# ASSERT-KTH/QuantizedSAE

Measured on AMD Instinct MI355X. Metric: activations/sec, BinarySAE 512->32768 n_bits=4 forward (dense latent + reconstruction + MSE), higher is better.
Workload: dtype f32; 1 GPU; BinarySAE(512, 32768, gamma=4.0, n_bits=4) k=65, 65536 rows per GPU per step, reference forward() signature (dense [B,32768] latent, [B,512] reconstruction, polarize loss) + recon-MSE accumulation; rows_per_gpu=65536, input_dim=512, hidden_dim=32768, n_bits=4, top_k=65, parallelism=row-sharded x1, no data-path collective, batches_in_flight=2

## Files before the change

### quantizedsae_amd/csrc/encode_topk_internal.h

```cpp
#pragma once

#include "gemm_mfma_f32_dma.h"
#include "decode_row.h"

namespace qsae {

int topk_rows_dispatch(float* latent, int64_t ld, int B, int H, int k, int32_t* idx, float* val, int zero_rest,
                       float* tau, uint2* cand, int* cnt, int cap, float* dense, int64_t dense_ld, hipStream_t s,
                       const float* margin = nullptr, int stride = 0);
int scatter_rows(const int32_t* idx, const float* val, int B, int k, int H, float* dense, int64_t ld, hipStream_t s);
int decode_binary_sparse_rows(const int* rows, int nrows, const int32_t* idx, const float* val, int k, int H,
                              const RowDecode& d, hipStream_t s);
int densify_rows(const int32_t* idx, const float* val, int B, int k, int H, float* dense, int64_t ld, hipStream_t s);
int gather_rows(const float* src, const int* rows, int n, int D, float* dst, hipStream_t s);
void launch_x_prep(const float* x, int B, int D, const float* meta, _Float16* xq, float* inv, float* margin, hipStream_t s,
                   int* zero_word = nullptr);

constexpr int kChunkRows = 1024;
constexpr int kTopkMaxH = 32768;
constexpr int kCandCap = 1024;
constexpr int kMaxSpecRows = kChunkRows;
constexpr int kRefMaxD = 2048;
constexpr int kRefTileStride = 36;

#ifdef QSAE_DEBUG_BUILD
#define QSAE_TUNABLE int
#define QSAE_TUNABLE_PTR unsigned long long*
extern int kPilotRank, g_xstat_rot, g_ref_ablate, g_ref_sliced, g_x_phase;
extern unsigned long long* g_ref_stamps;
#else
#define QSAE_TUNABLE static constexpr int
#define QSAE_TUNABLE_PTR static constexpr unsigned long long*
#endif
#if !defined(QSAE_DEBUG_BUILD) || defined(QSAE_DEFINE_SHARED_TUNABLES)
QSAE_TUNABLE kPilotRank = 20;
QSAE_TUNABLE g_xstat_rot = 2;
QSAE_TUNABLE_PTR g_ref_stamps = nullptr;
QSAE_TUNABLE g_ref_ablate = 0;
#ifdef QSAE_AB_NO_SLICED
QSAE_TUNABLE g_ref_sliced = 0;
#else
QSAE_TUNABLE g_ref_sliced = 1;
#endif
QSAE_TUNABLE g_x_phase = 3;
#endif

static inline size_t align_up(size_t v, size_t a) { return (v + a - 1) / a * a; }
bool use_fused(int B, int D, int H, int k);
int pilot_width(int H);

struct FusedLayout {
    size_t pilot, tau, cnt, cnt_split, cand, flags, fx, flat, fidx, fval, fpart, total;
};
FusedLayout fused_layout(int B, int D, int H, int k);

template <int BM, int BN, int WMW = 2, int WNW = 2, bool APPROX = false>
struct EpiFilter : EpiTile<BM, BN, WMW, WNW> {
    using T = EpiTile<BM, BN, WMW, WNW>;
    static constexpr int MT = T::MT, NT = T::NT;
    static constexpr int kThreads = 64 * WMW * WNW;
    static constexpr int kLdsFloats = BN;
    static constexpr int kStoresPerFinish = (BM * BN * 4) / (kThreads * 16);
    struct Args {
        const float* bias;
        const float* tau;
        uint2* cand;
        int* cnt;
        int cap;
        int hidden_offset;
        float* dense;
        int64_t dense_ld;
        const float* inv;
        const float* margin;
        int parts = 1;
        int* cnt_parts = nullptr;
    };
    float tau[NT];
    float inv[NT];
    bool col_ok[NT];

    __device__ __forceinline__ void begin(const Args& a, const TileCtx& c) {
        int* counters = reinterpret_cast<int*>(c.lds_epi);
        if (c.tid < BN) {
            const int row = c.n0 + c.tid;
            counters[c.tid] = (row < c.N && c.part == 0) ? a.cnt[row] : 0;
        }
#pragma unroll
        for (int nt = 0; nt < NT; ++nt) {
            const int col = T::col(c, nt);
            col_ok[nt] = col < c.N;
            tau[nt] = col_ok[nt] ? a.tau[col] : __builtin_huge_valf();
            inv[nt] = 1.0f;
            if (APPROX && col_ok[nt]) {
                tau[nt] = tau[nt] - a.margin[col];
                inv[nt] = a.inv[col];
            }
        }
    }
    __device__ __forceinline__ void init(const Args& a, f32x16 (&acc)[MT][NT], const TileCtx& c) {
#pragma unroll
        for (int mt = 0; mt < MT; ++mt)
#pragma unroll
            for (int r = 0; r < 16; ++r) {
                int h = T::row(c, mt, r);
                h = h < c.M ? h : c.M - 1;
                const float b = (!APPROX && a.bias) ? a.bias[h] : 0.0f;
#pragma unroll
                for (int nt = 0; nt < NT; ++nt) acc[mt][nt][r] = b;
            }
    }
    __device__ __forceinline__ void finish(const Args& a, f32x16 (&acc)[MT][NT], const TileCtx& c) {
        int* counters = reinterpret_cast<int*>(c.lds_epi);
        if (a.dense != nullptr) {
            constexpr int CPR = BM / 4;
            const int h0 = c.m0 + a.hidden_offset;
            const f32x4 z = {0.f, 0.f, 0.f, 0.f};
#pragma unroll
            for (int i = 0; i < (BN * CPR) / kThreads; ++i) {
                const int chunk = i * kThreads + c.tid;
                const int row = c.n0 + chunk / CPR, cc = 4 * (chunk % CPR);
                if (row < c.N && (c.m0 + cc) < c.M)
                    *reinterpret_cast<f32x4*>(a.dense + static_cast<int64_t>(row) * a.dense_ld + h0 + cc) = z;
            }
        }
        float hb[MT][16];
        if (APPROX) {
// ... 56 lines not shown
```

### quantizedsae_amd/csrc/prefilter_topk.hip

```cpp
#ifdef QSAE_DEBUG_BUILD
#define QSAE_DEFINE_SHARED_TUNABLES 1
#endif
#include "encode_topk_internal.h"
#include "sweep_xstat_f16.h"
#include "refine_row.h"
#include "refine_sliced.h"

namespace qsae {

constexpr int kFillCoWaves = 1024;
constexpr int kFillCoPace = 3;

QSAE_TUNABLE_PTR g_xstat_stamps = nullptr;
QSAE_TUNABLE g_fuse_xprep = 0;
QSAE_TUNABLE g_inkernel_pilot = 1;
QSAE_TUNABLE g_inkernel_rank = 0;
QSAE_TUNABLE g_pilot_tile = 0;
QSAE_TUNABLE g_fill_in_sweep = 1;
QSAE_TUNABLE g_fill_co = 1;
QSAE_TUNABLE g_xstat_ablate = 0;
QSAE_TUNABLE g_x_parts = 0;
QSAE_TUNABLE g_pref_tile = 2;

struct PrefLayout {
    size_t xq, inv, margin, cnt_parts, sl_offs, total_extra;
};
static PrefLayout pref_layout(int B, int D, size_t base) {
    PrefLayout P;
    size_t off = base;
    P.xq = off;     off = align_up(off + static_cast<size_t>(B) * D * 2, 256);
    P.inv = off;    off = align_up(off + static_cast<size_t>(B) * 4, 256);
    P.margin = off; off = align_up(off + static_cast<size_t>(B) * 4, 256);
    P.cnt_parts = off; off = align_up(off + static_cast<size_t>(B) * 4 * 7, 256);
    P.sl_offs = off; off = align_up(off + static_cast<size_t>(B) * 65, 256);
    P.total_extra = off;
    return P;
}

__global__ void __launch_bounds__(256)
pref_w_stats_kernel(const float* __restrict__ W, const float* __restrict__ bias, int H, int D, unsigned* __restrict__ meta) {
    const int row = blockIdx.x * 4 + (threadIdx.x >> 6), lane = threadIdx.x & 63;
    if (row >= H) return;
    float mx = 0.f, ss = 0.f;
    for (int d = lane; d < D; d += 64) pref_w_stat_step(W[static_cast<int64_t>(row) * D + d], mx, ss);
    pref_w_stat_join(mx, ss);
    if (lane == 0) {
        const float nrm = pref_w_row_norm(ss);
        atomicMax(&meta[1], __float_as_uint(nrm));
        atomicMax(&meta[3], __float_as_uint(mx));
        if (bias) atomicMax(&meta[2], __float_as_uint(fabsf(bias[row])));
    }
}

__global__ void __launch_bounds__(256)
pref_w_cast_kernel(const float* __restrict__ W, long long n, float* __restrict__ meta, _Float16* __restrict__ Wq) {
    const float sw = pow2_scale_for(meta[3]);
    const long long gid = static_cast<long long>(blockIdx.x) * blockDim.x + threadIdx.x;
    if (gid == 0) meta[0] = sw;
    if (gid < n) Wq[gid] = pref_w_cast(W[gid], sw);
}

__global__ void __launch_bounds__(256)
pref_w_err_kernel(const float* __restrict__ W, int H, int D, const float* __restrict__ sw_ptr, unsigned* __restrict__ out) {
    const int row = blockIdx.x * 4 + (threadIdx.x >> 6), lane = threadIdx.x & 63;
    if (row >= H) return;
    const float sw = *sw_ptr;
    if (!(sw > 0.f)) return;
    const float back = 1.0f / sw;
    float ff = 0.f;
    for (int d = lane; d < D; d += 64) pref_w_err_step(W[static_cast<int64_t>(row) * D + d], sw, back, ff);
    ff = pref_w_err_join(ff);
    if (lane == 0) atomicMax(out, __float_as_uint(pref_w_row_err(ff)));
}

template <int NV>
__global__ void __launch_bounds__(256)
pref_x_prep_kernel(const float* __restrict__ x, int B, int D, const float* __restrict__ meta,
                   _Float16* __restrict__ xq, float* __restrict__ inv, float* __restrict__ margin, int* __restrict__ zero_word) {
    const int row = blockIdx.x * 4 + (threadIdx.x >> 6), lane = threadIdx.x & 63;
    if (zero_word && blockIdx.x == 0 && threadIdx.x == 0) *zero_word = 0;
    if (row >= B) return;
    const float* xr = x + static_cast<int64_t>(row) * D;
    _Float16* qr = xq + static_cast<int64_t>(row) * D;
    float mx = 0.f, ss = 0.f;
    f32x4 keep[NV > 0 ? NV : 1];
    if (NV > 0) {
#pragma unroll
        for (int j = 0; j < NV; ++j) keep[j] = *reinterpret_cast<const f32x4*>(xr + 256 * j + 4 * lane);
#pragma unroll
        for (int j = 0; j < NV; ++j)
#pragma unroll
            for (int e = 0; e < 4; ++e) {
                const float v = keep[j][e], a = fabsf(v);
                mx = (a > mx || a != a) ? a : mx;
                ss = fmaf(v, v, ss);
            }
    } else {
        for (int d = lane; d < D; d += 64) {
            const float v = xr[d];
            const float a = fabsf(v);
            mx = (a > mx || a != a) ? a : mx;
            ss = fmaf(v, v, ss);
        }
    }
    for (int off = 32; off > 0; off >>= 1) {
        const float o = __shfl_xor(mx, off, 64);
        mx = (o > mx || o != o) ? o : mx;
        ss += __shfl_xor(ss, off, 64);
    }
    const float sx0 = pow2_scale_for(mx), back = sx0 > 0.f ? 1.0f / sx0 : 0.f;
    float ee = 0.f;
    if (NV > 0) {
#pragma unroll
        for (int j = 0; j < NV; ++j) {
            typedef _Float16 f16x4 __attribute__((ext_vector_type(4)));
            f16x4 q;
#pragma unroll
// ... 195 lines not shown
    const SweepProfile prof = take_sweep_profile();
    const PrefPlan pl = pref_plan(c);
    const FusedLayout& L = pl.L;
    const PrefLayout& PL = pl.PL;
    const int B = c.B, D = c.D, H = c.H, k = c.k, P = pl.P;
    char* ws = c.ws;
    float* pilot = reinterpret_cast<float*>(ws + L.pilot);
    float* tau = reinterpret_cast<float*>(ws + L.tau);
    int* cnt = reinterpret_cast<int*>(ws + L.cnt);
    uint2* cand = reinterpret_cast<uint2*>(ws + L.cand);
    int* flags = reinterpret_cast<int*>(ws + L.flags);
    _Float16* xq = reinterpret_cast<_Float16*>(ws + PL.xq);
    float* inv = reinterpret_cast<float*>(ws + PL.inv);
    float* margin = reinterpret_cast<float*>(ws + PL.margin);
    int* cnt_parts = reinterpret_cast<int*>(ws + PL.cnt_parts);
    const bool xstat = pl.xstat, inkernel = pl.inkernel, fill_co = pl.fill_co, fill_in_sweep = pl.fill_in_sweep;
    float* fused_fill = xstat ? nullptr : c.dense;
    const int Hs = pl.Hs, hoff = pl.hoff, parts = pl.parts, cap_part = pl.cap_part;
    const int xs_iters = xstat ? (Hs / kXsHT) / parts + (inkernel ? P / kXsHT : 0) : 0;
    const int fill_cw = xs_iters > 0 ? (32 * (H / 256) / parts + xs_iters - 1) / xs_iters : 0;
    ThreadDeviceCtx* ctx = nullptr;
    if (fill_co) {
        const int rc0 = thread_device_ctx(&ctx);
        if (rc0 != QSAE_OK) return rc0;
    }
    const bool fuse_prep = inkernel && g_fuse_xprep;
    if (!fuse_prep && (g_x_phase & 1)) {
        launch_x_prep(c.x, B, D, c.meta, xq, inv, margin, s, flags);
        QSAE_LAUNCH_CHECK();
    } else {
        QSAE_HIP(hipMemsetAsync(flags, 0, sizeof(int), s));
    }
    const int Kw = D / 2;
    const float* xq_w = reinterpret_cast<const float*>(xq);
    const float* wq_w = reinterpret_cast<const float*>(c.Wq);
    int rc = QSAE_OK;
    if (!inkernel) {
        if (g_pilot_tile == 0 && P % 256 == 0) {
            using EpiP = EpiApproxDense<256, 256, 4, 2>;
            typename EpiP::Args ep{inv, c.bias, pilot, P};
            rc = launch_gemm_dma<EpiP, 256, 256, true, 2>(xq_w, B, wq_w, P, Kw, ep, s, 8);
        } else {
            using EpiP = EpiApproxDense<256, 128, 4, 2>;
            typename EpiP::Args ep{inv, c.bias, pilot, P};
            rc = launch_gemm_dma<EpiP, 256, 128, true>(xq_w, B, wq_w, P, Kw, ep, s, 8);
        }
        if (rc != QSAE_OK) return rc;
    }
    const int j = kPilotRank < P ? kPilotRank : P;
    if (!inkernel) rc = topk_rows_dispatch(pilot, P, B, P, j, nullptr, nullptr, 0, tau, cand, cnt, cap_part, fused_fill, c.dense_ld, s,
                                margin, kCandCap);
    if (rc != QSAE_OK) return rc;
    if (g_x_phase & 1) {
        using EpiS = EpiFilter<256, 128, 4, 2, true>;
        typename EpiS::Args es{c.bias ? c.bias + P : nullptr, tau, cand, cnt, kCandCap, P, fused_fill, c.dense_ld, inv, margin};
        if (prof.begin) QSAE_HIP(hipEventRecord(prof.begin, s));
        if (xstat) {
            XsArgs xa{};
            xa.xq = xq;  xa.wq = c.Wq + static_cast<size_t>(hoff) * D;  xa.bias = c.bias ? c.bias + hoff : nullptr;  xa.tau = tau;
            xa.margin = margin;  xa.inv = inv;  xa.cand = cand;  xa.cnt = cnt;  xa.B = B;  xa.Hs = Hs;  xa.cap = kCandCap;
            xa.hidden_offset = hoff;  xa.rot_mul = g_xstat_rot;  xa.stamps = g_xstat_stamps;  xa.H = H;  xa.fill_cw = fill_cw;
            xa.dense = fill_in_sweep ? c.dense : nullptr;  xa.dense_ld = c.dense_ld;  xa.pilot_stages = inkernel ? P / kXsHT : 0;
            xa.pilot_rank = g_inkernel_rank > 0 ? g_inkernel_rank : inkernel_rank(k);  xa.tau_out = tau;  xa.meta = c.meta;
            xa.x32 = fuse_prep ? c.x : nullptr;  xa.inv_out = inv;  xa.margin_out = margin;  xa.parts = parts;  xa.cnt_parts = cnt_parts;
            if (fill_co) QSAE_HIP(hipEventRecord(ctx->ev_fork, s));
            rc = launch_xstat(D, xa, s, (g_xstat_ablate == 0 && D == 512 && !fill_in_sweep) ? 9 : g_xstat_ablate);
            if (fill_co && rc == QSAE_OK) rc = launch_fill_co(ctx, c.dense, c.dense_ld, B, H, s);
        } else if (g_pref_tile != 1) {
            using EpiW = EpiFilter<256, 256, 4, 2, true>;
            typename EpiW::Args ew{es.bias, es.tau, es.cand, es.cnt, es.cap, es.hidden_offset, es.dense, es.dense_ld, es.inv,
                                   es.margin};
            rc = launch_gemm_dma<EpiW, 256, 256, true, 2>(wq_w + static_cast<size_t>(P) * Kw, H - P, xq_w, B, Kw, ew, s);
        } else {
            rc = launch_gemm_dma<EpiS, 256, 128, true>(wq_w + static_cast<size_t>(P) * Kw, H - P, xq_w, B, Kw, es, s);
        }
        if (prof.end) QSAE_HIP(hipEventRecord(prof.end, s));
        if (rc != QSAE_OK) return rc;
        if (xstat && g_xstat_ablate != 0) return QSAE_OK;
    }
    if (g_x_phase & 2) {
        const RowDecode rd = c.dec ? *c.dec : RowDecode{nullptr, 0, 0, 0, 0, 0.f, nullptr, nullptr, nullptr};
        if (refine_sliced_wanted(B, D, H, k))
            return launch_refine_sliced(cand, cnt, tau, margin, c.x, c.W, c.bias, B, D, H, k, c.idx, c.val, flags, pl.filled, c.dense_ld,
                                        parts, cnt_parts, reinterpret_cast<uint8_t*>(ws + PL.sl_offs), rd, s);
        return launch_refine_row(cand, cnt, tau, margin, c.x, c.W, c.bias, B, D, H, k, c.idx, c.val, flags, pl.filled, c.dense_ld, parts,
                                 cnt_parts, rd, s);
    }
    QSAE_LAUNCH_CHECK();
    return QSAE_OK;
}

static FlaggedArgs pref_flagged_args(const PrefCall& c, const PrefPlan& pl) {
    return FlaggedArgs{c.x, c.W, c.bias, c.B, c.D, c.H, c.k, c.idx, c.val, c.ws, pl.L, c.stream, false,
                       pl.filled, c.dense_ld};
}

static int prefilter_finish(const PrefCall& c, int first, int nflag) {
    hipStream_t s = as_stream(c.stream);
    const PrefPlan pl = pref_plan(c);
    if (pl.xstat && g_xstat_ablate != 0) return QSAE_OK;
    if (nflag < 0 || nflag > c.B) return fail(QSAE_ERR_INVALID_ARG, "%s: flagged-row count out of range", __func__);
    int rc = flagged_range(pref_flagged_args(c, pl), first, nflag);
    if (rc != QSAE_OK) return rc;
    if (c.dec && nflag > 0) {
        const int* flags = reinterpret_cast<const int*>(c.ws + pl.L.flags);
        rc = decode_binary_sparse_rows(flags + 1, nflag, c.idx, c.val, c.k, c.H, *c.dec, s);
        if (rc != QSAE_OK) return rc;
    }
    if (c.dense && !pl.filled)
        return pl.xstat ? densify_rows(c.idx, c.val, c.B, c.k, c.H, c.dense, c.dense_ld, s)
                        : scatter_rows(c.idx, c.val, c.B, c.k, c.H, c.dense, c.dense_ld, s);
    return QSAE_OK;
}

static int run_prefilter(const PrefCall& c, int spec, int* flagged_rows) {
    int rc = prefilter_submit(c);
    if (rc != QSAE_OK) return rc;
    const PrefPlan pl = pref_plan(c);
    if (pl.xstat && g_xstat_ablate != 0) return QSAE_OK;
    const FlaggedArgs fa = pref_flagged_args(c, pl);
    int nflag = 0;
    hipStream_t s = as_stream(c.stream);
    {
        const int* flags = reinterpret_cast<const int*>(c.ws + pl.L.flags);
        ThreadDeviceCtx* ctx = nullptr;
        rc = thread_device_ctx(&ctx);
        if (rc != QSAE_OK) return rc;
        *ctx->pinned = 0;
        QSAE_HIP(hipMemcpyAsync(ctx->pinned, flags, sizeof(int), hipMemcpyDeviceToHost, s));
        QSAE_HIP(hipEventRecord(ctx->ev_copied, s));
        spec = spec < 0 ? 0 : (spec > kMaxSpecRows ? kMaxSpecRows : spec);
        spec = spec < c.B ? spec : c.B;
        rc = flagged_spec(fa, spec);
        if (rc != QSAE_OK) return rc;
        QSAE_HIP(hipEventSynchronize(ctx->ev_copied));
        nflag = *ctx->pinned;
    }
    if (flagged_rows) *flagged_rows = nflag;
    return prefilter_finish(c, spec, nflag);
}

}

using namespace qsae;

#ifdef QSAE_DEBUG_BUILD
namespace qsae { extern int g_pilot_div, g_force_path, g_sweep_kernel; }
extern "C" int qsae_debug_set_xstat_stamps(void* buf) {
    g_xstat_stamps = static_cast<unsigned long long*>(buf);
    return QSAE_OK;
}

extern "C" int qsae_debug_set_refine_stamps(void* buf) {
    g_ref_stamps = static_cast<unsigned long long*>(buf);
    return QSAE_OK;
}

extern "C" int qsae_debug_set_refine_sliced(int v) {
    g_ref_sliced = v;
    return QSAE_OK;
}

extern "C" int qsae_debug_set_refine_ablate(int v) {
    g_ref_ablate = v;
    return QSAE_OK;
}

extern "C" int qsae_debug_set_pilot(int div, int rank) {
    g_pilot_div = div;
    kPilotRank = rank;
    return QSAE_OK;
}

extern "C" int qsae_debug_set_inkernel_pilot(int enable, int rank) {
    g_fuse_xprep = enable >= 2 ? 1 : 0;
    enable = enable ? 1 : 0;
    g_inkernel_pilot = enable;
    g_inkernel_rank = rank;
    return QSAE_OK;
}

extern "C" int qsae_debug_set_fill_co(int v) {
    g_fill_co = v;
    return QSAE_OK;
}

extern "C" int qsae_debug_set_xstat_rot(int rot) {
    g_pilot_tile = rot >= 1000 ? 1 : 0;
    rot %= 1000;
    g_fill_in_sweep = rot >= 100 ? 0 : 1;
    rot %= 100;
    g_xstat_rot = rot;
    return QSAE_OK;
}

extern "C" int qsae_debug_set_prefilter_tile(int which) {
    g_xstat_ablate = which >= 10 ? which - 10 : 0;
    g_pref_tile = which >= 10 ? 2 : which;
    return QSAE_OK;
}

extern "C" int qsae_debug_set_phases(int phase_mask, int parts) {
    g_x_phase = phase_mask;
    g_x_parts = parts;
    return QSAE_OK;
}

extern "C" int qsae_debug_set_sweep_kernel(int which) {
    g_sweep_kernel = which;
    return QSAE_OK;
}

extern "C" int qsae_debug_set_topk_path(int path) {
    g_force_path = path;
    return QSAE_OK;
}

extern "C" int qsae_debug_prefilter_offsets(int B, int D, int H, int k, size_t* pilot_off, size_t* margin_off,
                                            int* pilot_cols) {
    const FusedLayout L = fused_layout(B, D, H, k);
    const PrefLayout PL = pref_layout(B, D, L.total);
    if (pilot_off) *pilot_off = L.pilot;
    if (margin_off) *margin_off = PL.margin;
    if (pilot_cols) *pilot_cols = pilot_width(H);
    return QSAE_OK;
}

extern "C" int qsae_debug_prefilter_list_offsets(int B, int D, int H, int k, size_t* cand_off, size_t* cnt_off,
                                                 size_t* cnt_parts_off, size_t* tau_off, size_t* margin_off, int* cap,
                                                 int* parts) {
    const FusedLayout L = fused_layout(B, D, H, k);
    const PrefLayout PL = pref_layout(B, D, L.total);
    if (cand_off) *cand_off = L.cand;
    if (cnt_off) *cnt_off = L.cnt;
    if (cnt_parts_off) *cnt_parts_off = PL.cnt_parts;
    if (tau_off) *tau_off = L.tau;
    if (margin_off) *margin_off = PL.margin;
    if (cap) *cap = kCandCap;
    if (parts) *parts = xstat_parts(B, H, kCandCap);
    return QSAE_OK;
}
#endif

extern "C" double qsae_profile_sweep_flop_fraction(int H) {
    if (H <= 0) return 0.0;
    if (g_inkernel_pilot && g_pref_tile == 2 && H % kXsHT == 0 && pilot_width(H) % kXsHT == 0) return 1.0;
    return static_cast<double>(H - pilot_width(H)) / static_cast<double>(H);
}

extern "C" size_t qsae_prefilter_w_bytes(int H, int D) {
    return (H > 0 && D > 0) ? static_cast<size_t>(H) * D * 2 : 0;
}

extern "C" int qsae_prefilter_pack_w(const float* W, const float* bias, int H, int D, void* Wq, float* meta,
                                     qsae_stream_t stream) {
    QSAE_CHECK_ARG(H > 0 && D > 0 && W && Wq && meta, "H > 0, D > 0, non-null pointers");
    hipStream_t s = as_stream(stream);
    QSAE_HIP(hipMemsetAsync(meta, 0, 4 * sizeof(float), s));
    hipLaunchKernelGGL(pref_w_stats_kernel, dim3((H + 3) / 4), dim3(256), 0, s, W, bias, H, D,
                       reinterpret_cast<unsigned*>(meta));
    QSAE_LAUNCH_CHECK();
    const long long n = static_cast<long long>(H) * D;
    hipLaunchKernelGGL(pref_w_cast_kernel, dim3(static_cast<unsigned>((n + 255) / 256)), dim3(256), 0, s, W, n, meta,
                       static_cast<_Float16*>(Wq));
    QSAE_LAUNCH_CHECK();
    QSAE_HIP(hipMemsetAsync(meta + 3, 0, sizeof(float), s));
    hipLaunchKernelGGL(pref_w_err_kernel, dim3((H + 3) / 4), dim3(256), 0, s, W, H, D, meta, reinterpret_cast<unsigned*>(meta + 3));
    QSAE_LAUNCH_CHECK();
    return QSAE_OK;
}

extern "C" size_t qsae_encode_topk_prefilter_workspace_bytes(int B, int D, int H, int k) {
    if (B <= 0 || H <= 0 || D <= 0 || k <= 0 || !prefilter_shape_ok(B, D, H, k)) return 0;
    return pref_layout(B, D, fused_layout(B, D, H, k).total).total_extra;
}

static int prefilter_call(const char* who, const float* x, const float* W, const float* bias, const void* Wq, const float* meta,
                          int B, int D, int H, int k, const uint8_t* packed, int n_bits, float step, const float* dec_bias,
                          int32_t* idx, float* val, float* dense, int64_t dense_ld, float* recon, void* workspace,
                          size_t workspace_bytes, qsae_stream_t stream, PrefCall& call, RowDecode& dec,
                          const float* table = nullptr) {
    if (!(x && W && Wq && meta && idx && val && workspace)) return fail(QSAE_ERR_INVALID_ARG, "%s: invalid argument: null pointer", who);
    if (!(k >= 1 && k <= H)) return fail(QSAE_ERR_INVALID_ARG, "%s: invalid argument: 1 <= k <= H required", who);
    if (!prefilter_shape_ok(B, D, H, k))
        return fail(QSAE_ERR_UNSUPPORTED, "%s: unsupported: shape outside the prefilter's range (use qsae_encode_topk_latent)", who);
    if (workspace_bytes < qsae_encode_topk_prefilter_workspace_bytes(B, D, H, k))
        return fail(QSAE_ERR_WORKSPACE, "%s: workspace too small", who);
    if (!(aligned16(workspace) && aligned16(x) && aligned16(W) && aligned16(Wq)))
        return fail(QSAE_ERR_INVALID_ARG, "%s: invalid argument: 16-byte alignment", who);
    if (dense && !(dense_ld >= H && dense_ld % 4 == 0 && aligned16(dense)))
        return fail(QSAE_ERR_INVALID_ARG, "%s: invalid argument: dense latent alignment / ld", who);
    call = PrefCall{x, W, bias, static_cast<const _Float16*>(Wq), meta, B, D, H, k, idx, val, static_cast<char*>(workspace),
                    stream, dense, dense_ld, nullptr};
    if (packed) {
        if (!recon) return fail(QSAE_ERR_INVALID_ARG, "%s: invalid argument: packed given without recon", who);
        if (!(n_bits >= 1 && n_bits <= 8)) return fail(QSAE_ERR_INVALID_ARG, "%s: invalid argument: 1 <= n_bits <= 8 required", who);
        if ((reinterpret_cast<uintptr_t>(packed) & 3u) != 0)
            return fail(QSAE_ERR_INVALID_ARG, "%s: invalid argument: packed must be 4-byte aligned", who);
        dec = RowDecode{reinterpret_cast<const uint32_t*>(packed), qsae_binary_row_bytes(D, n_bits) / 4, n_bits,
                        field_width(n_bits), D, step, dec_bias, recon, nullptr};
        call.dec = &dec;
    } else if (table) {
        if (!recon) return fail(QSAE_ERR_INVALID_ARG, "%s: invalid argument: table given without recon", who);
        if (!(aligned16(table) && aligned16(recon)))
            return fail(QSAE_ERR_INVALID_ARG, "%s: invalid argument: table and recon must be 16-byte aligned", who);
        dec = RowDecode{nullptr, 0, 0, 0, D, step, dec_bias, recon, table};
        call.dec = &dec;
    }
    return QSAE_OK;
}

enum class PrefMode { blocking, submit, finish };
static int prefilter_entry(const char* who, PrefMode mode, bool need_dict, const float* x, const float* W, const float* bias,
                           const void* Wq, const float* meta, int B, int D, int H, int k, const uint8_t* packed, int n_bits, float step,
                           const float* table, const float* dec_bias, int32_t* idx, float* val, float* dense, int64_t dense_ld,
                           float* recon, void* workspace, size_t workspace_bytes, int n, int* out, qsae_stream_t stream) {
    if (!(B >= 0 && D > 0 && H > 0)) return fail(QSAE_ERR_INVALID_ARG, "%s: invalid argument: B >= 0, D > 0, H > 0 required", who);
    if (mode == PrefMode::submit && !out)
        return fail(QSAE_ERR_INVALID_ARG, "%s: invalid argument: flagged_host must point to a host int", who);
    if (out && (mode == PrefMode::blocking || B == 0)) *out = 0;
    if (B == 0) return QSAE_OK;
    if (need_dict && !((packed || table) && recon)) return fail(QSAE_ERR_INVALID_ARG, "%s: invalid argument: null pointer", who);
// ... 74 lines not shown
```

### quantizedsae_amd/csrc/refine_sliced.h

```cpp
#pragma once

#include "refine_row.h"

namespace qsae {

constexpr int kSlList = 256;
constexpr int kSlMaxSlices = 64;
constexpr int kSlRowsPerWave = 128;
constexpr int kSlXRows = 24;
constexpr int kSlQueue = 512;
constexpr int kSlicedMinK = 48;
constexpr int kSlicedMinRows = 8192;
static_assert(kSlList * 8 <= kCandCap * 8, "sorted list + values must fit the row's candidate segment");
constexpr int kSlSelectLds = kCandCap * 4 + kCandCap * 2 + kRefMaxSurv * 4;
constexpr int kSlSelectLdsNoIdx = kCandCap * 4 + kRefMaxSurv * 4;
constexpr int kSlChainLds = 64 * 32 * 4 + kSlXRows * kRefTileStride * 4 + kSlQueue * 2 + 32 * 4;
constexpr int kSlRankLds = kRefMaxSurv * 8 + 2 * kRefMaxSurv * 4 + kRefMaxSurv * 4;

template <bool kIdxInLds>
__global__ void __launch_bounds__(64 * kRefWaves)
refine_select_kernel(uint2* __restrict__ cand, const int* __restrict__ cnt, int cap, const float* __restrict__ tau,
                     const float* __restrict__ margin, int B, int H, int k, int parts, const int* __restrict__ cnt_parts,
                     int* __restrict__ flags, int S, int per_shift, uint8_t* __restrict__ offs ) {
    extern __shared__ __attribute__((aligned(16))) unsigned char sel_smem[];
    const int lane = threadIdx.x & 63;
    const int wave = __builtin_amdgcn_readfirstlane(threadIdx.x >> 6);
    const int b = blockIdx.x * kRefWaves + wave;
    if (b >= B) return;
    constexpr int kLds = kIdxInLds ? kSlSelectLds : kSlSelectLdsNoIdx;
    float* wt = reinterpret_cast<float*>(sel_smem + static_cast<size_t>(wave) * kLds);
    int* hidx = reinterpret_cast<int*>(sel_smem + static_cast<size_t>(wave) * kLds + (kIdxInLds ? kCandCap * 6 : kCandCap * 4));
    auto flag_row = [&]() {
        if (lane == 0) {
            const int slot = atomicAdd(&flags[0], 1);
            flags[1 + slot] = b;
        }
    };
    auto no_stamp = [](int) {};
    auto no_survivors = [&]() {
        for (int s = lane; s <= S; s += 64) offs[static_cast<size_t>(s) * B + b] = 0;
    };
    float tau_b, margin_b;
    int m = refine_select_row<kIdxInLds>(cand, cnt, cap, tau, margin, B, H, k, parts, cnt_parts, b, lane, wt, hidx, flag_row, no_stamp,
                                         tau_b, margin_b);
    if (m > 255) { flag_row(); m = -1; }
    if (m < 0) { no_survivors(); return; }
    asm volatile("" ::: "memory");
    const int nsl = (m + 63) / 64;
    int mine[4];
    bool unordered = false;
    int last_slice = 0;
#pragma unroll
    for (int t = 0; t < 4; ++t) {
        const int j = 64 * t + lane;
        mine[t] = 0x7FFFFFFF;
        if (t < nsl) {
            if (j < m) mine[t] = hidx[j];
            const int sl = mine[t] >> per_shift;
            int before = __shfl_up(sl, 1, 64);
            before = lane == 0 ? last_slice : before;
            unordered |= j < m && sl < before;
            last_slice = __builtin_amdgcn_readlane(sl, 63);
        }
    }
    int* list = reinterpret_cast<int*>(cand + static_cast<int64_t>(b) * cap);
    if (!__any(unordered)) {
#pragma unroll
        for (int t = 0; t < 4; ++t)
            if (t < nsl && 64 * t + lane < m) list[64 * t + lane] = mine[t];
    } else {
        int pos[4];
        bool twice = false;
#pragma unroll
        for (int t = 0; t < 4; ++t) {
            pos[t] = -1;
            if (t < nsl && 64 * t + lane < m) {
                int below = 0, same = 0;
                for (int i = 0; i < m; ++i) {
                    const int o = hidx[i];
                    below += (o < mine[t]) ? 1 : 0;
                    same += (o == mine[t]) ? 1 : 0;
                }
                pos[t] = below;
                twice |= same != 1;
            }
        }
        if (__any(twice)) { flag_row(); no_survivors(); return; }
#pragma unroll
        for (int t = 0; t < 4; ++t)
            if (pos[t] >= 0) list[pos[t]] = mine[t];
    }
    const int per = 1 << per_shift;
    int myoff = 0;
    for (int s = 1; s < S; ++s) {
        const int lim = s * per;
        int c = 0;
#pragma unroll
        for (int t = 0; t < 4; ++t)
            if (t < nsl) c += __popcll(__ballot(mine[t] < lim));
        if (lane == s) myoff = c;
    }
    if (lane < S) offs[static_cast<size_t>(lane) * B + b] = static_cast<uint8_t>(myoff);
    if (lane == 0) offs[static_cast<size_t>(S) * B + b] = static_cast<uint8_t>(m);
}

template <int NXL>
__device__ __forceinline__ void slice_chain_batch(const float* __restrict__ x, const float* __restrict__ W, const float* __restrict__ bias,
                                                  uint2* __restrict__ cand, int cap, int D, int row0, uint32_t my, bool valid, int lane,
                                                  float* wt, float* xt, const int* xr, int R, int rx, int h) {
// ... 26 lines not shown
#pragma unroll
        for (int i = 0; i < 8; ++i) sv[i] = *reinterpret_cast<const f32x4*>(wb + woff[i] + 128 * blk);
#pragma unroll
        for (int i = 0; i < NXL; ++i) sv[8 + i] = *reinterpret_cast<const f32x4*>(xb + xoff[i] + 128 * blk);
    };
    auto consume = [&](const f32x4 (&sv)[NL]) {
#pragma unroll
        for (int i = 0; i < 8; ++i) *reinterpret_cast<f32x4*>(wput + 256 * i) = sv[i];
#pragma unroll
        for (int i = 0; i < NXL; ++i) *reinterpret_cast<f32x4*>(xput + 8 * kRefTileStride * i) = sv[8 + i];
        asm volatile("" ::: "memory");
#pragma unroll
        for (int part = 0; part < 8 / kChunks; ++part) {
            f32x4 w[kChunks], xv[kChunks];
#pragma unroll
            for (int q = 0; q < kChunks; ++q) {
                w[q] = *reinterpret_cast<const f32x4*>(wrow + 4 * ((kChunks * part + q) ^ wkey));
                xv[q] = *reinterpret_cast<const f32x4*>(xrow_t + 4 * (kChunks * part + q));
            }
#pragma unroll
            for (int q = 0; q < kChunks; ++q) {
                acc = fmaf(xv[q][0], w[q][0], acc);
                acc = fmaf(xv[q][1], w[q][1], acc);
                acc = fmaf(xv[q][2], w[q][2], acc);
                acc = fmaf(xv[q][3], w[q][3], acc);
            }
            asm volatile("" : "+v"(acc) :: "memory");
        }
    };
    auto issue = [&](f32x4 (&sv)[NL], int blk) {
        const char* sw = wb + 128 * blk;
        const char* sx = xb + 128 * blk;
#pragma unroll
        for (int i = 0; i < 8; ++i) asm volatile("global_load_dwordx4 %0, %1, %2" : "=&v"(sv[i]) : "v"(woff[i]), "s"(sw));
#pragma unroll
        for (int i = 0; i < NXL; ++i) asm volatile("global_load_dwordx4 %0, %1, %2" : "=&v"(sv[8 + i]) : "v"(xoff[i]), "s"(sx));
    };
#define QSAE_SL_REGS8 "+v"(sv[0]), "+v"(sv[1]), "+v"(sv[2]), "+v"(sv[3]), "+v"(sv[4]), "+v"(sv[5]), "+v"(sv[6]), "+v"(sv[7])
    auto landed = [&](f32x4 (&sv)[NL]) {
        if (NXL == 1) asm volatile("s_waitcnt vmcnt(9)" : QSAE_SL_REGS8, "+v"(sv[8]));
        else if (NXL == 2) asm volatile("s_waitcnt vmcnt(10)" : QSAE_SL_REGS8, "+v"(sv[8]), "+v"(sv[NL - 1]));
        else asm volatile("s_waitcnt vmcnt(11)" : QSAE_SL_REGS8, "+v"(sv[8]), "+v"(sv[9]), "+v"(sv[NL - 1]));
    };
    auto all_landed = [&](f32x4 (&sv)[NL]) {
        if (NXL == 1) asm volatile("s_waitcnt vmcnt(0)" : QSAE_SL_REGS8, "+v"(sv[8]));
        else if (NXL == 2) asm volatile("s_waitcnt vmcnt(0)" : QSAE_SL_REGS8, "+v"(sv[8]), "+v"(sv[NL - 1]));
        else asm volatile("s_waitcnt vmcnt(0)" : QSAE_SL_REGS8, "+v"(sv[8]), "+v"(sv[9]), "+v"(sv[NL - 1]));
    };
#undef QSAE_SL_REGS8
    static_assert(NXL == 1 || NXL == 2 || NXL == 3, "wait counts above");
    int t = 0;
    if (nblk >= kSets) {
#pragma unroll
        for (int q = 0; q < kSets; ++q) issue(st[q], q);
        asm volatile("" : "+v"(acc));
        for (; t + 2 * kSets <= nblk; t += kSets) {
#pragma unroll
            for (int q = 0; q < kSets; ++q) {
                landed(st[q]);
                consume(st[q]);
                issue(st[q], t + q + kSets);
            }
        }
#pragma unroll
        for (int q = 0; q < kSets; ++q) all_landed(st[q]);
    } else {
#pragma unroll
        for (int q = 0; q < kSets; ++q)
            if (q < nblk) visible_load(st[q], q);
    }
    for (; t < nblk; t += kSets) {
#pragma unroll
        for (int q = 0; q < kSets; ++q) {
            if (t + q < nblk) {
                consume(st[q]);
                if (t + q + kSets < nblk) visible_load(st[q], t + q + kSets);
            }
        }
    }
    if (valid) reinterpret_cast<float*>(list)[kSlList + ent] = acc;
}
static_assert(kSlXRows == 24, "slice_chain_batch<3> fills exactly 24 tile rows");

__global__ void __launch_bounds__(64 * kRefWaves, 3)
refine_slice_chain_kernel(const float* __restrict__ x, const float* __restrict__ W, const float* __restrict__ bias,
                          uint2* __restrict__ cand, int cap, const uint8_t* __restrict__ offs, int B, int D, int S) {
    extern __shared__ __attribute__((aligned(16))) unsigned char chain_smem[];
    const int lane = threadIdx.x & 63;
    const int wave = __builtin_amdgcn_readfirstlane(threadIdx.x >> 6);
    unsigned char* base = chain_smem + static_cast<size_t>(wave) * kSlChainLds;
    float* wt = reinterpret_cast<float*>(base);
    float* xt = wt + 64 * 32;
    uint16_t* queue = reinterpret_cast<uint16_t*>(xt + kSlXRows * kRefTileStride);
    int* xr = reinterpret_cast<int*>(queue + kSlQueue);
    const int g = blockIdx.x, xcd = g & 7, q = g >> 3;
    const int wgs_per_slice = (B + kSlRowsPerWave * kRefWaves - 1) / (kSlRowsPerWave * kRefWaves);
    const int slice = xcd + 8 * (q / wgs_per_slice);
    if (slice >= S) return;
    const int row0 = ((q % wgs_per_slice) * kRefWaves + wave) * kSlRowsPerWave;
    if (row0 >= B) return;
    int at[2], left[2];
#pragma unroll
    for (int half = 0; half < 2; ++half) {
        const int r = row0 + 64 * half + lane;
        at[half] = 0;
        left[half] = 0;
        if (r < B) {
            at[half] = offs[static_cast<size_t>(slice) * B + r];
            left[half] = static_cast<int>(offs[static_cast<size_t>(slice + 1) * B + r]) - at[half];
        }
    }
    while (__any(left[0] > 0 || left[1] > 0)) {
        int total = 0;
#pragma unroll
        for (int half = 0; half < 2; ++half) {
            const int c = left[half];
            int incl = c;
            for (int off = 1; off < 64; off <<= 1) {
                const int o = __shfl_up(incl, off, 64);
                if (lane >= off) incl += o;
            }
            const int start = total + incl - c;
            int wrote = 0;
            for (int i = 0; i < c; ++i)
                if (start + i < kSlQueue) {
                    queue[start + i] = static_cast<uint16_t>(((64 * half + lane) << 8) | (at[half] + i));
                    ++wrote;
                }
            at[half] += wrote;
            left[half] -= wrote;
            total += __shfl(incl, 63, 64);
        }
        total = total < kSlQueue ? total : kSlQueue;
        asm volatile("" ::: "memory");
        auto pair_h = [&](uint32_t q) {
            const int* l = reinterpret_cast<const int*>(cand + static_cast<int64_t>(row0 + static_cast<int>(q >> 8)) * cap);
            return l[q & 255u];
        };
        int p0 = 0;
        int h_next = pair_h(queue[lane < total ? lane : 0]);
        while (p0 < total) {
            const int p = p0 + lane;
            const bool in = p < total;
            const uint32_t my = queue[in ? p : p0];
            const int h_now = h_next;
            const int rl = static_cast<int>(my >> 8);
            const int prev = __shfl_up(rl, 1, 64);
            const bool head = in && (lane == 0 || prev != rl);
            const unsigned long long hb = __ballot(head);
            int rx = __popcll(hb & ((2ull << lane) - 1ull)) - 1;
            const unsigned long long over = __ballot(in && rx >= kSlXRows);
            const int take = over ? __builtin_ctzll(over) : (total - p0 < 64 ? total - p0 : 64);
            const bool valid = lane < take;
            const int R = __popcll(hb & (take >= 64 ? ~0ull : ((1ull << take) - 1ull)));
            if (head && valid) xr[rx] = row0 + rl;
            rx = valid ? rx : 0;
            asm volatile("" ::: "memory");
            {
                const int pn = p0 + take + lane;
                const uint32_t qn = queue[pn < total ? pn : (p0 + take < total ? p0 + take : 0)];
                h_next = pair_h(qn);
            }
            if (R <= 8) slice_chain_batch<1>(x, W, bias, cand, cap, D, row0, my, valid, lane, wt, xt, xr, R, rx, h_now);
            else if (R <= 16) slice_chain_batch<2>(x, W, bias, cand, cap, D, row0, my, valid, lane, wt, xt, xr, R, rx, h_now);
            else slice_chain_batch<3>(x, W, bias, cand, cap, D, row0, my, valid, lane, wt, xt, xr, R, rx, h_now);
            asm volatile("" ::: "memory");
            p0 += take;
        }
    }
}

template <int kDecode>
__global__ void __launch_bounds__(64 * kRefWaves, kDecode == 0 ? 3 : 4)
refine_rank_kernel(const uint2* __restrict__ cand, int cap, const uint8_t* __restrict__ offs, int S, int B, int k,
                   int32_t* __restrict__ idx_out, float* __restrict__ val_out, int* __restrict__ flags, float* __restrict__ dense,
                   int64_t dense_ld, RowDecode dec) {
    extern __shared__ __attribute__((aligned(16))) unsigned char rank_smem[];
    const int lane = threadIdx.x & 63;
    const int wave = __builtin_amdgcn_readfirstlane(threadIdx.x >> 6);
    const int b = blockIdx.x * kRefWaves + wave;
    if (b >= B) return;
    const int m = offs[static_cast<size_t>(S) * B + b];
    if (m == 0) return;
    unsigned char* mybase = rank_smem + static_cast<size_t>(wave) * kSlRankLds;
    unsigned long long* ekey = reinterpret_cast<unsigned long long*>(mybase);
    float* wt = reinterpret_cast<float*>(mybase + kRefMaxSurv * 8);
    int* hval = reinterpret_cast<int*>(wt + 2 * kRefMaxSurv);
    const int* list = reinterpret_cast<const int*>(cand + static_cast<int64_t>(b) * cap);
    for (int j = lane; j < m; j += 64) {
        const int h = list[j];
        const float v = reinterpret_cast<const float*>(list)[kSlList + j];
        ekey[j] = full_key(v, static_cast<uint32_t>(h));
        reinterpret_cast<float*>(hval)[j] = v;
    }
    asm volatile("" ::: "memory");
    auto no_stamp = [](int) {};
    refine_rank_decode<kDecode>(ekey, hval, wt, m, k, b, lane, idx_out, val_out, dense, dense_ld, flags, dec, no_stamp);
}

static bool sliced_plan(int H, int D, int* S, int* shift) {
    int sh = 0;
    while ((static_cast<size_t>(2) << sh) * D * 4 <= (4u << 20)) ++sh;
    int n = (H + (1 << sh) - 1) >> sh;
    n = (n + 7) / 8 * 8;
    *S = n;
    *shift = sh;
    return n <= kSlMaxSlices;
}

static bool sliced_fits(int H, int D) {
    int S, sh;
    return sliced_plan(H, D, &S, &sh);
}

static bool refine_sliced_wanted(int B, int D, int H, int k) {
    return g_ref_sliced != 0 && g_ref_ablate == 0 && g_ref_stamps == nullptr && D % 32 == 0 && D / 32 >= 2 &&
           static_cast<uint64_t>(H) * D * 4 < (1ull << 32) && static_cast<uint64_t>(B) * D * 4 < (1ull << 32) &&
           (g_ref_sliced == 2 || (B >= kSlicedMinRows && k >= kSlicedMinK)) && sliced_fits(H, D);
}

static int launch_refine_sliced(uint2* cand, const int* cnt, const float* tau, const float* margin, const float* x, const float* W,
                                const float* bias, int B, int D, int H, int k, int32_t* idx, float* val, int* flags, float* filled,
                                int64_t dense_ld, int parts, const int* cnt_parts, uint8_t* offs, const RowDecode& rd, hipStream_t s) {
    int S = 0, per_shift = 0;
    sliced_plan(H, D, &S, &per_shift);
    QSAE_SET_MAX_LDS_ONCE(refine_select_kernel<true>, 160 * 1024);
    QSAE_SET_MAX_LDS_ONCE(refine_slice_chain_kernel, 160 * 1024);
    const dim3 rows_grid((B + kRefWaves - 1) / kRefWaves), block(64 * kRefWaves);
    if (!(g_x_phase & 8)) {
        if (parts == 1)
            hipLaunchKernelGGL(refine_select_kernel<false>, rows_grid, block, kSlSelectLdsNoIdx * kRefWaves, s, cand, cnt, kCandCap,
                               tau, margin, B, H, k, parts, cnt_parts, flags, S, per_shift, offs);
        else
            hipLaunchKernelGGL(refine_select_kernel<true>, rows_grid, block, kSlSelectLds * kRefWaves, s, cand, cnt, kCandCap, tau,
                               margin, B, H, k, parts, cnt_parts, flags, S, per_shift, offs);
        QSAE_LAUNCH_CHECK();
        const int wgs_per_slice = (B + kSlRowsPerWave * kRefWaves - 1) / (kSlRowsPerWave * kRefWaves);
        hipLaunchKernelGGL(refine_slice_chain_kernel, dim3(8 * (S / 8) * wgs_per_slice), block, kSlChainLds * kRefWaves, s, x,
                           W, bias, cand, kCandCap, offs, B, D, S);
        QSAE_LAUNCH_CHECK();
    }
    if (g_x_phase & 4) return QSAE_OK;
    auto rank = refine_rank_kernel<0>;
    if (!rd.active()) rank = refine_rank_kernel<3>;
    else if (rd.packed && !rd.table && rd.fw == 4) rank = refine_rank_kernel<1>;
    else if (rd.packed && !rd.table && rd.fw == 8) rank = refine_rank_kernel<2>;
    hipLaunchKernelGGL(rank, rows_grid, block, kSlRankLds * kRefWaves, s, cand, kCandCap, offs, S, B, k, idx, val, flags, filled,
                       dense_ld, rd);
    QSAE_LAUNCH_CHECK();
    return QSAE_OK;
}

}
```

Measured before the change: 17.77 million activations/s.

## Schedule slice-chain refine work via persistent workgroups pulling from atomic task queues

Replaces the fixed one-workgroup-per-(slice,row-block) grid of the slice chain kernel with a capped persistent grid whose waves pull (slice, row-group) tasks from eight per-XCD atomic counters. Each wave steals from other queues after finishing its home queue. The select kernel now zeroes these counters. The goal is to balance uneven per-slice candidate loads and cut tail idle time. Shuffles are also swapped for ds_bpermute/readlane intrinsics. The atomics add contention, and queue ordering may hurt cache locality.

```diff
diff --git a/quantizedsae_amd/csrc/encode_topk_internal.h b/quantizedsae_amd/csrc/encode_topk_internal.h
--- a/quantizedsae_amd/csrc/encode_topk_internal.h
+++ b/quantizedsae_amd/csrc/encode_topk_internal.h
@@ -26,7 +26,7 @@
 #ifdef QSAE_DEBUG_BUILD
 #define QSAE_TUNABLE int
 #define QSAE_TUNABLE_PTR unsigned long long*
-extern int kPilotRank, g_xstat_rot, g_ref_ablate, g_ref_sliced, g_x_phase;
+extern int kPilotRank, g_xstat_rot, g_ref_ablate, g_ref_sliced, g_x_phase, g_sl_grid_cap, g_sl_rows, g_sl_split;
 extern unsigned long long* g_ref_stamps;
 #else
 #define QSAE_TUNABLE static constexpr int
@@ -42,6 +42,9 @@
 #else
 QSAE_TUNABLE g_ref_sliced = 1;
 #endif
+QSAE_TUNABLE g_sl_grid_cap = 0;
+QSAE_TUNABLE g_sl_rows = 128;
+QSAE_TUNABLE g_sl_split = 0;
 QSAE_TUNABLE g_x_phase = 3;
 #endif
 
diff --git a/quantizedsae_amd/csrc/prefilter_topk.hip b/quantizedsae_amd/csrc/prefilter_topk.hip
--- a/quantizedsae_amd/csrc/prefilter_topk.hip
+++ b/quantizedsae_amd/csrc/prefilter_topk.hip
@@ -23,7 +23,7 @@
 QSAE_TUNABLE g_pref_tile = 2;
 
 struct PrefLayout {
-    size_t xq, inv, margin, cnt_parts, sl_offs, total_extra;
+    size_t xq, inv, margin, cnt_parts, sl_offs, sl_ctr, total_extra;
 };
 static PrefLayout pref_layout(int B, int D, size_t base) {
     PrefLayout P;
@@ -33,6 +33,7 @@
     P.margin = off; off = align_up(off + static_cast<size_t>(B) * 4, 256);
     P.cnt_parts = off; off = align_up(off + static_cast<size_t>(B) * 4 * 7, 256);
     P.sl_offs = off; off = align_up(off + static_cast<size_t>(B) * 65, 256);
+    P.sl_ctr = off; off = align_up(off + static_cast<size_t>(kSlQueues) * kSlCtrStride * 4, 256);
     P.total_extra = off;
     return P;
 }
@@ -394,7 +395,7 @@
         const RowDecode rd = c.dec ? *c.dec : RowDecode{nullptr, 0, 0, 0, 0, 0.f, nullptr, nullptr, nullptr};
         if (refine_sliced_wanted(B, D, H, k))
             return launch_refine_sliced(cand, cnt, tau, margin, c.x, c.W, c.bias, B, D, H, k, c.idx, c.val, flags, pl.filled, c.dense_ld,
-                                        parts, cnt_parts, reinterpret_cast<uint8_t*>(ws + PL.sl_offs), rd, s);
+                                        parts, cnt_parts, reinterpret_cast<uint8_t*>(ws + PL.sl_offs), reinterpret_cast<int*>(ws + PL.sl_ctr), rd, s);
         return launch_refine_row(cand, cnt, tau, margin, c.x, c.W, c.bias, B, D, H, k, c.idx, c.val, flags, pl.filled, c.dense_ld, parts,
                                  cnt_parts, rd, s);
     }
@@ -473,6 +474,15 @@
     return QSAE_OK;
 }
 
+extern "C" int qsae_debug_set_chain_grid(int max_workgroups, int task_rows, int split_rounds) {
+    if (max_workgroups < 0 || !(task_rows == 0 || task_rows == 32 || task_rows == 64 || task_rows == 128))
+        return fail(QSAE_ERR_INVALID_ARG, "%s: max_workgroups >= 0, task_rows 0, 32, 64 or 128", __func__);
+    g_sl_grid_cap = max_workgroups;
+    g_sl_rows = task_rows ? task_rows : kSlRowsPerWave;
+    g_sl_split = split_rounds ? 1 : 0;
+    return QSAE_OK;
+}
+
 extern "C" int qsae_debug_set_refine_ablate(int v) {
     g_ref_ablate = v;
     return QSAE_OK;
@@ -550,6 +560,17 @@
     if (margin_off) *margin_off = PL.margin;
     if (cap) *cap = kCandCap;
     if (parts) *parts = xstat_parts(B, H, kCandCap);
+    return QSAE_OK;
+}
+
+extern "C" int qsae_debug_sliced_offsets(int B, int D, int H, int k, size_t* offs_off, size_t* ctr_off, int* slices, int* list_ints) {
+    const PrefLayout PL = pref_layout(B, D, fused_layout(B, D, H, k).total);
+    int S = 0, shift = 0;
+    if (!sliced_plan(H, D, &S, &shift)) return fail(QSAE_ERR_UNSUPPORTED, "%s: more than %d slices", __func__, kSlMaxSlices);
+    if (offs_off) *offs_off = PL.sl_offs;
+    if (ctr_off) *ctr_off = PL.sl_ctr;
+    if (slices) *slices = S;
+    if (list_ints) *list_ints = kSlList;
     return QSAE_OK;
 }
 #endif
diff --git a/quantizedsae_amd/csrc/refine_sliced.h b/quantizedsae_amd/csrc/refine_sliced.h
--- a/quantizedsae_amd/csrc/refine_sliced.h
+++ b/quantizedsae_amd/csrc/refine_sliced.h
@@ -7,6 +7,9 @@
 constexpr int kSlList = 256;
 constexpr int kSlMaxSlices = 64;
 constexpr int kSlRowsPerWave = 128;
+constexpr int kSlQueues = 8;
+constexpr int kSlCtrStride = 32;
+constexpr int kSlChainGrid = 256 * 3;
 constexpr int kSlXRows = 24;
 constexpr int kSlQueue = 512;
 constexpr int kSlicedMinK = 48;
@@ -21,10 +24,12 @@
 __global__ void __launch_bounds__(64 * kRefWaves)
 refine_select_kernel(uint2* __restrict__ cand, const int* __restrict__ cnt, int cap, const float* __restrict__ tau,
                      const float* __restrict__ margin, int B, int H, int k, int parts, const int* __restrict__ cnt_parts,
-                     int* __restrict__ flags, int S, int per_shift, uint8_t* __restrict__ offs ) {
+                     int* __restrict__ flags, int S, int per_shift, uint8_t* __restrict__ offs ,
+                     int* __restrict__ task_ctr ) {
     extern __shared__ __attribute__((aligned(16))) unsigned char sel_smem[];
     const int lane = threadIdx.x & 63;
     const int wave = __builtin_amdgcn_readfirstlane(threadIdx.x >> 6);
+    if (blockIdx.x == 0 && threadIdx.x < kSlQueues) task_ctr[threadIdx.x * kSlCtrStride] = 0;
     const int b = blockIdx.x * kRefWaves + wave;
     if (b >= B) return;
     constexpr int kLds = kIdxInLds ? kSlSelectLds : kSlSelectLdsNoIdx;
@@ -217,42 +222,36 @@
 }
 static_assert(kSlXRows == 24, "slice_chain_batch<3> fills exactly 24 tile rows");
 
-__global__ void __launch_bounds__(64 * kRefWaves, 3)
-refine_slice_chain_kernel(const float* __restrict__ x, const float* __restrict__ W, const float* __restrict__ bias,
-                          uint2* __restrict__ cand, int cap, const uint8_t* __restrict__ offs, int B, int D, int S) {
-    extern __shared__ __attribute__((aligned(16))) unsigned char chain_smem[];
-    const int lane = threadIdx.x & 63;
-    const int wave = __builtin_amdgcn_readfirstlane(threadIdx.x >> 6);
-    unsigned char* base = chain_smem + static_cast<size_t>(wave) * kSlChainLds;
-    float* wt = reinterpret_cast<float*>(base);
-    float* xt = wt + 64 * 32;
-    uint16_t* queue = reinterpret_cast<uint16_t*>(xt + kSlXRows * kRefTileStride);
-    int* xr = reinterpret_cast<int*>(queue + kSlQueue);
-    const int g = blockIdx.x, xcd = g & 7, q = g >> 3;
-    const int wgs_per_slice = (B + kSlRowsPerWave * kRefWaves - 1) / (kSlRowsPerWave * kRefWaves);
-    const int slice = xcd + 8 * (q / wgs_per_slice);
-    if (slice >= S) return;
-    const int row0 = ((q % wgs_per_slice) * kRefWaves + wave) * kSlRowsPerWave;
-    if (row0 >= B) return;
-    int at[2], left[2];
-#pragma unroll
-    for (int half = 0; half < 2; ++half) {
+template <int kRows>
+__device__ __forceinline__ void slice_chain_task(const float* __restrict__ x, const float* __restrict__ W, const float* __restrict__ bias,
+                                                 uint2* __restrict__ cand, int cap, const uint8_t* __restrict__ offs, int B, int D,
+                                                 int slice, int row0, int lane, float* wt, float* xt, uint16_t* queue, int* xr) {
+    static_assert(kRows == 32 || kRows == 64 || kRows == 128, "a queue entry keeps 7 row bits; the rows of a task sit on lanes");
+    constexpr int kHalves = kRows > 64 ? 2 : 1;
+    int at[kHalves], left[kHalves];
+#pragma unroll
+    for (int half = 0; half < kHalves; ++half) {
         const int r = row0 + 64 * half + lane;
         at[half] = 0;
         left[half] = 0;
-        if (r < B) {
+        if (64 * half + lane < kRows && r < B) {
             at[half] = offs[static_cast<size_t>(slice) * B + r];
             left[half] = static_cast<int>(offs[static_cast<size_t>(slice + 1) * B + r]) - at[half];
         }
     }
-    while (__any(left[0] > 0 || left[1] > 0)) {
+    bool more = false;
+#pragma unroll
+    for (int half = 0; half < kHalves; ++half) more |= left[half] > 0;
+    while (__any(more)) {
         int total = 0;
-#pragma unroll
-        for (int half = 0; half < 2; ++half) {
+        int sl = lane;
+        asm volatile("" : "+v"(sl));
+#pragma unroll
+        for (int half = 0; half < kHalves; ++half) {
             const int c = left[half];
             int incl = c;
             for (int off = 1; off < 64; off <<= 1) {
-                const int o = __shfl_up(incl, off, 64);
+                const int o = __builtin_amdgcn_ds_bpermute((sl - off) << 2, incl);
                 if (lane >= off) incl += o;
             }
             const int start = total + incl - c;
@@ -264,7 +263,7 @@
                 }
             at[half] += wrote;
             left[half] -= wrote;
-            total += __shfl(incl, 63, 64);
+            total += __builtin_amdgcn_readlane(incl, 63);
         }
         total = total < kSlQueue ? total : kSlQueue;
         asm volatile("" ::: "memory");
@@ -275,32 +274,66 @@
         int p0 = 0;
         int h_next = pair_h(queue[lane < total ? lane : 0]);
         while (p0 < total) {
-            const int p = p0 + lane;
+            int bl = lane;
+            asm volatile("" : "+v"(bl));
+            const int p = p0 + bl;
             const bool in = p < total;
             const uint32_t my = queue[in ? p : p0];
             const int h_now = h_next;
             const int rl = static_cast<int>(my >> 8);
-            const int prev = __shfl_up(rl, 1, 64);
-            const bool head = in && (lane == 0 || prev != rl);
+            const int prev = __builtin_amdgcn_ds_bpermute((bl - 1) << 2, rl);
+            const bool head = in && (bl == 0 || prev != rl);
             const unsigned long long hb = __ballot(head);
-            int rx = __popcll(hb & ((2ull << lane) - 1ull)) - 1;
+            int rx = __popcll(hb & ((2ull << bl) - 1ull)) - 1;
             const unsigned long long over = __ballot(in && rx >= kSlXRows);
             const int take = over ? __builtin_ctzll(over) : (total - p0 < 64 ? total - p0 : 64);
-            const bool valid = lane < take;
+            const bool valid = bl < take;
             const int R = __popcll(hb & (take >= 64 ? ~0ull : ((1ull << take) - 1ull)));
             if (head && valid) xr[rx] = row0 + rl;
             rx = valid ? rx : 0;
             asm volatile("" ::: "memory");
             {
-                const int pn = p0 + take + lane;
+                const int pn = p0 + take + bl;
                 const uint32_t qn = queue[pn < total ? pn : (p0 + take < total ? p0 + take : 0)];
                 h_next = pair_h(qn);
             }
-            if (R <= 8) slice_chain_batch<1>(x, W, bias, cand, cap, D, row0, my, valid, lane, wt, xt, xr, R, rx, h_now);
-            else if (R <= 16) slice_chain_batch<2>(x, W, bias, cand, cap, D, row0, my, valid, lane, wt, xt, xr, R, rx, h_now);
-            else slice_chain_batch<3>(x, W, bias, cand, cap, D, row0, my, valid, lane, wt, xt, xr, R, rx, h_now);
+            if (R <= 8) slice_chain_batch<1>(x, W, bias, cand, cap, D, row0, my, valid, bl, wt, xt, xr, R, rx, h_now);
+            else if (R <= 16) slice_chain_batch<2>(x, W, bias, cand, cap, D, row0, my, valid, bl, wt, xt, xr, R, rx, h_now);
+            else slice_chain_batch<3>(x, W, bias, cand, cap, D, row0, my, valid, bl, wt, xt, xr, R, rx, h_now);
             asm volatile("" ::: "memory");
             p0 += take;
+        }
+        more = false;
+#pragma unroll
+        for (int half = 0; half < kHalves; ++half) more |= left[half] > 0;
+    }
+}
+
+template <int kRows>
+__global__ void __launch_bounds__(64 * kRefWaves, 3)
+refine_slice_chain_kernel(const float* __restrict__ x, const float* __restrict__ W, const float* __restrict__ bias,
+                          uint2* __restrict__ cand, int cap, const uint8_t* __restrict__ offs, int B, int D, int round0, int rounds,
+                          int* __restrict__ task_ctr) {
+    extern __shared__ __attribute__((aligned(16))) unsigned char chain_smem[];
+    const int lane = threadIdx.x & 63;
+    const int wave = __builtin_amdgcn_readfirstlane(threadIdx.x >> 6);
+    unsigned char* base = chain_smem + static_cast<size_t>(wave) * kSlChainLds;
+    float* wt = reinterpret_cast<float*>(base);
+    float* xt = wt + 64 * 32;
+    uint16_t* queue = reinterpret_cast<uint16_t*>(xt + kSlXRows * kRefTileStride);
+    int* xr = reinterpret_cast<int*>(queue + kSlQueue);
+    const int home = blockIdx.x & (kSlQueues - 1);
+    const int groups = (B + kRows - 1) / kRows;
+    const int per_queue = rounds * groups;
+    for (int turn = 0; turn < kSlQueues; ++turn) {
+        const int qi = (home + turn) & (kSlQueues - 1);
+        for (;;) {
+            int task = 0;
+            if (lane == 0) task = atomicAdd(&task_ctr[qi * kSlCtrStride], 1);
+            task = __builtin_amdgcn_readfirstlane(task);
+            if (task >= per_queue) break;
+            slice_chain_task<kRows>(x, W, bias, cand, cap, offs, B, D, qi + kSlQueues * (round0 + task / groups), (task % groups) * kRows,
+                                    lane, wt, xt, queue, xr);
         }
     }
 }
@@ -354,25 +387,50 @@
            (g_ref_sliced == 2 || (B >= kSlicedMinRows && k >= kSlicedMinK)) && sliced_fits(H, D);
 }
 
+template <int kRows>
+static void launch_slice_chains(const float* x, const float* W, const float* bias, uint2* cand, const uint8_t* offs, int B, int D,
+                                int round0, int rounds, int* task_ctr, hipStream_t s) {
+    const long long tasks = static_cast<long long>(kSlQueues) * rounds * ((B + kRows - 1) / kRows);
+    long long grid = (tasks + kRefWaves - 1) / kRefWaves;
+    grid = grid < kSlChainGrid ? grid : kSlChainGrid;
+    if (g_sl_grid_cap > 0 && grid > g_sl_grid_cap) grid = g_sl_grid_cap;
+    hipLaunchKernelGGL(refine_slice_chain_kernel<kRows>, dim3(static_cast<unsigned>(grid)), dim3(64 * kRefWaves),
+                       kSlChainLds * kRefWaves, s, x, W, bias, cand, kCandCap, offs, B, D, round0, rounds, task_ctr);
+}
+
 static int launch_refine_sliced(uint2* cand, const int* cnt, const float* tau, const float* margin, const float* x, const float* W,
                                 const float* bias, int B, int D, int H, int k, int32_t* idx, float* val, int* flags, float* filled,
-                                int64_t dense_ld, int parts, const int* cnt_parts, uint8_t* offs, const RowDecode& rd, hipStream_t s) {
+                                int64_t dense_ld, int parts, const int* cnt_parts, uint8_t* offs, int* task_ctr, const RowDecode& rd,
+                                hipStream_t s) {
     int S = 0, per_shift = 0;
     sliced_plan(H, D, &S, &per_shift);
     QSAE_SET_MAX_LDS_ONCE(refine_select_kernel<true>, 160 * 1024);
-    QSAE_SET_MAX_LDS_ONCE(refine_slice_chain_kernel, 160 * 1024);
+    QSAE_SET_MAX_LDS_ONCE(refine_slice_chain_kernel<kSlRowsPerWave>, 160 * 1024);
     const dim3 rows_grid((B + kRefWaves - 1) / kRefWaves), block(64 * kRefWaves);
     if (!(g_x_phase & 8)) {
         if (parts == 1)
             hipLaunchKernelGGL(refine_select_kernel<false>, rows_grid, block, kSlSelectLdsNoIdx * kRefWaves, s, cand, cnt, kCandCap,
-                               tau, margin, B, H, k, parts, cnt_parts, flags, S, per_shift, offs);
+                               tau, margin, B, H, k, parts, cnt_parts, flags, S, per_shift, offs, task_ctr);
         else
             hipLaunchKernelGGL(refine_select_kernel<true>, rows_grid, block, kSlSelectLds * kRefWaves, s, cand, cnt, kCandCap, tau,
-                               margin, B, H, k, parts, cnt_parts, flags, S, per_shift, offs);
+                               margin, B, H, k, parts, cnt_parts, flags, S, per_shift, offs, task_ctr);
         QSAE_LAUNCH_CHECK();
-        const int wgs_per_slice = (B + kSlRowsPerWave * kRefWaves - 1) / (kSlRowsPerWave * kRefWaves);
-        hipLaunchKernelGGL(refine_slice_chain_kernel, dim3(8 * (S / 8) * wgs_per_slice), block, kSlChainLds * kRefWaves, s, x,
-                           W, bias, cand, kCandCap, offs, B, D, S);
+#ifdef QSAE_DEBUG_BUILD
+        if (g_sl_rows != kSlRowsPerWave || g_sl_split) {
+            QSAE_SET_MAX_LDS_ONCE(refine_slice_chain_kernel<32>, 160 * 1024);
+            QSAE_SET_MAX_LDS_ONCE(refine_slice_chain_kernel<64>, 160 * 1024);
+            QSAE_SET_MAX_LDS_ONCE(refine_slice_chain_kernel<128>, 160 * 1024);
+            const int nl = g_sl_split ? S / 8 : 1, each = g_sl_split ? 1 : S / 8;
+            for (int l = 0; l < nl; ++l) {
+                if (l > 0) QSAE_HIP(hipMemsetAsync(task_ctr, 0, kSlQueues * kSlCtrStride * sizeof(int), s));
+                if (g_sl_rows == 32) launch_slice_chains<32>(x, W, bias, cand, offs, B, D, l * each, each, task_ctr, s);
+                else if (g_sl_rows == 64) launch_slice_chains<64>(x, W, bias, cand, offs, B, D, l * each, each, task_ctr, s);
+                else launch_slice_chains<128>(x, W, bias, cand, offs, B, D, l * each, each, task_ctr, s);
+                QSAE_LAUNCH_CHECK();
+            }
+        } else
+#endif
+        launch_slice_chains<kSlRowsPerWave>(x, W, bias, cand, offs, B, D, 0, S / 8, task_ctr, s);
         QSAE_LAUNCH_CHECK();
     }
     if (g_x_phase & 4) return QSAE_OK;
```

After: 17.27 million activations/s. -2.8%, worse.
